# HydrogenSulfate/LFT

Hardware: AMD Instinct MI355X
Metric: LF patches/sec (5x5 angRes, 32x32 LR, 4xSR) (higher is better)
Workload: dtype bf16; 1 GPU; LFT 5x5 angRes 4xSR inference, batch=4 per GPU, 32x32 LR patches; global_batch=4, parallelism=dp1 (independent shards), streams_per_gpu=1, hip_graph=True, steps_in_flight=2

## Files before the change

### lft_amd/_lib.py

```python
from __future__ import annotations

import ctypes
import os
import subprocess
from ctypes import POINTER, c_char_p, c_float, c_int, c_longlong, c_size_t, c_void_p

HERE = os.path.dirname(os.path.abspath(__file__))
CSRC = os.path.join(HERE, "csrc")
LIB_PATH = os.environ.get("LFT_LIB_PATH") or os.path.join(HERE, "liblft_hip.so")
SOURCES = ["lft_api.hip", "lft_common.cuh", "lft_kernels_a.cuh", "lft_kernels_b.cuh", "lft_train.cuh", "lft_train_host.cuh", "lft_attn_maps.cuh", "lft_metrics.cuh", "lft_prepare.cuh"]
ABI_VERSION = 5
STATUS_NONFINITE = 1001

PREC_F32, PREC_BF16, PREC_F16 = 0, 1, 2
MATH_F32, MATH_BF16X3, MATH_BF16X6 = 0, 1, 2
NUM_PARAMS = 78

_lib = None


class LftError(RuntimeError):
    pass


# ... 75 lines not shown
    "lft_bicubic_fwd": (c_int, [c_void_p, c_void_p, c_int, c_int, c_int, c_int, c_int, c_void_p]),
    "lft_init_features_fwd": (c_int, [c_void_p, c_void_p, c_void_p, c_void_p, c_int, c_int, c_int, c_int, c_int, c_int, c_void_p]),
    "lft_ang_block_fwd": (c_int, [c_void_p, c_int, c_void_p, c_void_p, c_int, c_int, c_int, c_int, c_int, c_int, c_void_p]),
    "lft_spa_block_fwd": (c_int, [c_void_p, c_int, c_void_p, c_void_p, c_void_p, c_void_p, c_int, c_int, c_int, c_int, c_int, c_int, c_void_p]),
    "lft_upsample_fwd": (c_int, [c_void_p, c_void_p, c_void_p, c_void_p, c_void_p, c_int, c_int, c_int, c_int, c_int, c_int, c_void_p]),
    "lft_scene_counts": (c_int, [c_int, c_int, c_int, c_int, POINTER(c_int), POINTER(c_int)]),
    "lft_scene_divide": (c_int, [c_void_p, c_void_p, c_int, c_int, c_int, c_int, c_int, c_void_p]),
    "lft_scene_integrate": (c_int, [c_void_p, c_void_p, c_int, c_int, c_int, c_int, c_int, c_int, c_void_p]),
    "lft_train_tape_bytes": (c_int, [c_int, c_int, c_int, c_int, c_int, POINTER(c_size_t)]),
    "lft_train_grad_floats": (c_int, [c_int, POINTER(c_size_t)]),
    "lft_train_tape_offset": (c_int, [c_char_p, c_int, c_int, c_int, c_int, c_int, POINTER(c_size_t)]),
    "lft_train_forward": (c_int, [POINTER(c_void_p), c_int, c_void_p, c_void_p, c_void_p, c_int, c_int, c_int, c_int, c_int, c_int, c_void_p]),
    "lft_train_backward": (c_int, [POINTER(c_void_p), c_int, c_void_p, c_void_p, c_void_p, c_void_p, c_int, c_int, c_int, c_int, c_int, c_int, c_void_p]),
    "lft_train_backward_input": (c_int, [POINTER(c_void_p), c_int, c_void_p, c_void_p, c_void_p, c_void_p, c_void_p,
                                         c_int, c_int, c_int, c_int, c_int, c_int, c_void_p]),
    "lft_lr_grad_bwd": (c_int, [c_void_p, c_void_p, c_void_p, c_void_p, c_int, c_int, c_int, c_int, c_int, c_void_p]),
    "lft_train_backward_buckets": (c_int, [POINTER(c_void_p), c_int, c_void_p, c_void_p, c_void_p, c_void_p, c_int, c_int, c_int, c_int, c_int, c_int,
                                           c_void_p, c_void_p, c_void_p]),
    "lft_train_block_backward": (c_int, [POINTER(c_void_p), c_int, c_void_p, c_void_p, c_int, c_int, c_void_p, c_void_p, c_void_p,
                                         c_int, c_int, c_int, c_int, c_int, c_int, c_void_p]),
    "lft_train_grad_bucket": (c_int, [c_int, c_int, POINTER(c_size_t), POINTER(c_size_t)]),
    "lft_train_step_profiled": (c_int, [POINTER(c_void_p), c_int, c_void_p, c_void_p, c_void_p, c_void_p, c_void_p, c_int, c_int, c_int, c_int, c_int, c_int,
                                        c_void_p, c_int, POINTER(c_float), POINTER(c_char_p), POINTER(c_int)]),
    "lft_attn_maps_floats": (c_int, [c_int, c_int, c_int, c_int, c_int, c_int, POINTER(c_size_t)]),
    "lft_train_attn_maps": (c_int, [c_void_p, c_int, c_int, c_int, c_void_p, c_int, c_int, c_int, c_int, c_int, c_void_p]),
    "lft_l1_loss": (c_int, [c_void_p, c_void_p, c_longlong, c_void_p, c_float, c_void_p, c_void_p, c_void_p]),
    "lft_adam_step": (c_int, [c_void_p, c_void_p, c_void_p, c_void_p, c_longlong, c_float, c_float, c_float, c_float, c_int, c_float, c_float, c_void_p]),
    "lft_view_metrics_scratch_bytes": (c_int, [c_int, c_int, c_int, c_int, POINTER(c_size_t)]),
    "lft_view_metrics": (c_int, [c_void_p, c_void_p, c_int, c_int, c_int, c_int, c_float, c_void_p, c_void_p, c_void_p, c_void_p]),
    "lft_lf_prepare": (c_int, [c_void_p, c_int, c_int, c_int, c_int, c_int, c_int, POINTER(c_longlong), c_int, c_int,
                               POINTER(c_int), c_int, c_int, c_int, c_void_p, c_void_p, c_int, c_void_p, c_void_p, c_int,
                               c_void_p, c_void_p, c_void_p]),
    "lft_mfma_selftest": (c_int, [c_void_p, c_void_p, c_void_p, c_void_p, c_void_p, c_int, c_void_p]),
}
EXPORTS = tuple(_SIGS)
TEST_EXPORTS = ("lft_mfma_selftest",)
BLOCK_UPSAMPLE, BLOCK_SPA, BLOCK_ANG, BLOCK_INIT = 0, 1, 2, 3
LF_UINT8, LF_FLOAT32, LF_FLOAT64 = 0, 1, 2
MAPS_MEAN, MAPS_HEADS = 0, 1
GRAD_BUCKETS = 3
BUCKET_FN = ctypes.CFUNCTYPE(c_int, c_void_p, c_int, c_size_t, c_size_t)


def lib() -> ctypes.CDLL:
    global _lib
    if _lib is None:
        if not os.path.exists(LIB_PATH):
            raise LftError(f"{LIB_PATH} is missing: the HIP extension has not been built "
                           "(run __graft_entry__.build()); there is no CPU fallback")
        L = ctypes.CDLL(LIB_PATH)
        L.lft_version.restype, L.lft_version.argtypes = c_int, []
        got = L.lft_version()
        if got != ABI_VERSION:
            raise LftError(f"{LIB_PATH} reports ABI version {got}, this binding needs {ABI_VERSION}: rebuild it (__graft_entry__.build())")
        for name, (res, args) in _SIGS.items():
            fn = getattr(L, name)
            fn.restype, fn.argtypes = res, args
        _lib = L
    return _lib


def check(rc: int, what: str) -> None:
    if rc != 0:
        msg = lib().lft_last_error()
        raise LftError(f"{what} failed (code {rc}): {msg.decode() if msg else ''}")


def packed_bytes(A, h, w, s, prec) -> int:
    n = c_size_t(0)
    check(lib().lft_packed_bytes(A, h, w, s, prec, ctypes.byref(n)), "lft_packed_bytes")
    return n.value


def workspace_bytes(B, A, h, w, s, prec) -> int:
    n = c_size_t(0)
    check(lib().lft_workspace_bytes(B, A, h, w, s, prec, ctypes.byref(n)), "lft_workspace_bytes")
    return n.value
```

### lft_amd/csrc/lft_api.hip

```cpp
#include "../../include/lft_hip.h"
#include "../../include/lft_hip_test.h"
#include <hip/hip_runtime.h>
#include <stdint.h>

#include <cstdarg>
#include <cstdio>
#include <cmath>
#include <set>
#include <string>
#include <algorithm>
#include <type_traits>
#include <utility>
#include <vector>

#ifndef LFT_TU
#define LFT_TU 0
#endif

namespace {
#include "lft_kernels_a.cuh"
#include "lft_kernels_b.cuh"
#include "lft_metrics.cuh"
#include "lft_prepare.cuh"
#include "lft_train.cuh"
// ... 85 lines not shown
    return fail(LFT_ERR_ARG, "internal: no kernel variant for %d", (int)v);
}
template <int V> using int_c = std::integral_constant<int, V>;
template <typename F> int by_prec(int prec, F&& f) {
    if (prec == LFT_PREC_F32) return f(float{});
    if (prec == LFT_PREC_BF16) return f(bf16_t{});
    return f(f16_t{});
}
inline size_t align256(size_t x) { return (x + 255) & ~(size_t)255; }

struct Dims {
    int B, A, V, h, w, hw, s, gp, gt, nchunk;
    long long ntok;
};

int make_dims(int B, int A, int h, int w, int s, int prec, Dims* d) {
    if (prec != LFT_PREC_F32 && prec != LFT_PREC_BF16 && prec != LFT_PREC_F16)
        return fail(LFT_ERR_ARG, "prec must be LFT_PREC_F32, LFT_PREC_BF16 or LFT_PREC_F16, got %d", prec);
    if (B < 1 || A < 1 || h < 1 || w < 1) return fail(LFT_ERR_SHAPE, "B, A, h, w must be positive (B=%d A=%d h=%d w=%d)", B, A, h, w);
    if (s != 2 && s != 4) return fail(LFT_ERR_SHAPE, "scale factor must be 2 or 4, got %d", s);
    if (A * A > 128) return fail(LFT_ERR_UNSUPPORTED, "angRes %d (A*A=%d views > 128) is not implemented in this build", A, A * A);
    if ((long long)B * A * A * h * w > (1LL << 27)) return fail(LFT_ERR_SHAPE, "too many tokens");
    d->B = B; d->A = A; d->V = A * A; d->h = h; d->w = w; d->hw = h * w; d->s = s;
    d->gp = (s + 2) * (s + 2); d->gt = (d->gp + 31) / 32; d->nchunk = 2 * s * s;
    d->ntok = (long long)B * d->V * d->hw;
    return 0;
}

constexpr int kFragsConv = 72, kFragsAng = 64, kFragsSpa1 = 240, kFragsSpa1NoQ = 208, kFragsSpa2 = 176;
inline int frags_up(const Dims& d) { return d.nchunk * (4 + 2 * d.gt); }

struct PackedLayout {
    size_t conv0_w, ln_ang[kLayers], ln_spa[kLayers], ang_pe, petok[kLayers], spa_pe_img;
    size_t s_conv[3], s_ang[kLayers], s_spa1[kLayers], s_spa2[kLayers], s_up, total;
};

PackedLayout packed_layout(const Dims& d, int prec) {
    const size_t esz = prec == LFT_PREC_F32 ? 4 : 2, fragb = 64 * 8 * esz;
    PackedLayout L;
    size_t o = 0;
    auto take = [&](size_t bytes) { size_t r = o; o = align256(o + bytes); return r; };
    L.conv0_w = take(576 * 4);
    for (int l = 0; l < kLayers; ++l) { L.ln_ang[l] = take(256 * 4); L.ln_spa[l] = take(512 * 4); }
    L.ang_pe = take((size_t)((d.V + 31) / 32) * 2048 * 4);
    for (int l = 0; l < kLayers; ++l) L.petok[l] = take((size_t)((d.hw + 32 * kNwSpa1 - 1) / (32 * kNwSpa1)) * kNwSpa1 * 4096 * esz);
    L.spa_pe_img = take((size_t)d.hw * 64 * esz);
    for (int i = 0; i < 3; ++i) L.s_conv[i] = take(kFragsConv * fragb);
    for (int l = 0; l < kLayers; ++l) {
        L.s_ang[l] = take(kFragsAng * fragb);
        L.s_spa1[l] = take(kFragsSpa1 * fragb);
        L.s_spa2[l] = take(kFragsSpa2 * fragb);
    }
    L.s_up = take((size_t)frags_up(d) * fragb);
    L.total = o;
    return L;
}

struct WorkLayout {
    size_t x0, feat, xa, xb, tok, q, k, v, o, g, status, total;
};
WorkLayout work_layout(const Dims& d, int prec) {
    const size_t esz = prec == LFT_PREC_F32 ? 4 : 2;
    WorkLayout W;
    size_t o = 0;
    auto take = [&](size_t bytes) { size_t r = o; o = align256(o + bytes); return r; };
    const size_t n = (size_t)d.ntok;
    W.x0 = take(n * 64 * esz); W.feat = take(n * 64 * esz); W.xa = take(n * 64 * esz); W.xb = take(n * 64 * esz);
    W.tok = take(n * 128 * esz); W.q = take(n * 128 * esz); W.k = take(n * 128 * esz); W.v = take(n * 128 * esz);
    W.o = take(n * 128 * esz);
    W.g = take(n * d.gp * 4);
    W.status = take(256);
    W.total = o;
    return W;
}

template <typename T> size_t lds_conv64(int w) { return WRing<T, kConv64Chunk, kNwConv>::LDS_BYTES + ConvIn<T, kNwConv>::bytes(w) + kNwConv * TileIO<2, T>::BYTES + kConvZeroRow; }
constexpr size_t kLdsParams = 1024;
template <typename T, int CH = kSpaChunk> size_t lds_spa1(int w) {
    return WRing<T, CH, kNwSpa1>::LDS_BYTES + std::max<size_t>(ConvIn<T, kNwSpa1>::bytes(w), (size_t)kNwSpa1 * TileIO<4, T>::BYTES) + kLdsParams + kConvZeroRow;
}
template <typename T> size_t lds_spa2() { return WRing<T, kSpaChunk, kNwSpa2>::LDS_BYTES + kLdsParams + kNwSpa2 * TileIO<4, T>::BYTES; }
template <typename T> size_t lds_up() { return WRing<T, kUpChunk, kNwUp>::LDS_BYTES + kNwUp * TileIO<2, T>::BYTES; }
template <typename T> size_t lds_ang() { return (size_t)kFragsAng * 1024 * FragInfo<T>::PIECES + kLdsParams + 4 * TileIO<2, T>::BYTES; }
constexpr size_t kMaxLds = 160 * 1024;
template <typename K> int allow_lds(K kernel, size_t bytes, const char* name) {
    if (bytes > kMaxLds) return fail(LFT_ERR_SHAPE, "%s needs %zu B of LDS (> 160 KiB): view width too large for this build", name, bytes);
    if (bytes <= 64 * 1024) return 0;
    struct Done { int dev; const void* fn; size_t bytes; };
    static thread_local std::vector<Done> done;
    const void* fn = reinterpret_cast<const void*>(kernel);
    int dev = 0;
    LFT_HIP_OK(hipGetDevice(&dev));
    for (const auto& d : done)
        if (d.dev == dev && d.fn == fn && d.bytes >= bytes) return 0;
    LFT_HIP_OK(hipFuncSetAttribute(fn, hipFuncAttributeMaxDynamicSharedMemorySize, (int)bytes));
    done.push_back(Done{dev, fn, bytes});
    return 0;
}

template <typename P> P* at(const void* base, size_t off) { return reinterpret_cast<P*>(const_cast<char*>(static_cast<const char*>(base)) + off); }
inline unsigned blocks_for(long long items, int per_block) { return (unsigned)((items + per_block - 1) / per_block); }

PackOp lin_op(const float* src, int row0, int nrows, int ld, int k0, int ksteps, int kmap, float scale, int kmul = 1, int kadd = 0) {
    PackOp p{};
    p.src = src; p.kind = 0; p.row0 = row0; p.nrows = nrows; p.ntiles = (nrows + 31) / 32; p.ld = ld;
    p.kmul = kmul; p.kadd = kadd; p.k0 = k0; p.ksteps = ksteps; p.kmap = kmap; p.scale = scale; p.s = 0; p.frag0 = 0;
    return p;
}
void conv_ops(std::vector<PackOp>& v, const float* w, int nout) {
// ... 25 lines not shown
template <typename T> bool tok_lane_major(const Dims& d) {
    return d.hw % (32 * kNwSpa1) == 0 && (sizeof(T) == 4 || d.w % 32 == 0);
}
template <typename T, bool PE_ONLY>
int launch_spa1(unsigned nwg, const T* in, const T* ws, const float* ln, const T* petok, T* tok, T* q, T* k, T* v, T* pe_out,
                int nimg, const Dims& d, hipStream_t st, unsigned* status) {
    const size_t l16 = lds_spa1<T, 16>(d.w), l8 = lds_spa1<T, 8>(d.w);
    const size_t share = kMaxLds / kSpaOcc;
    const bool use8 = (l16 > share && l8 <= share) || l16 > kMaxLds;
    const bool lm = !PE_ONLY && tok_lane_major<T>(d);
    return dispatch<8, 16>(use8 ? 8 : 16, [&](auto CH) {
        return dispatch<true, false>(lm, [&](auto LM) {
            constexpr bool WQ = !(LM && sizeof(T) == 2);
            const size_t lds = CH == 8 ? l8 : l16;
            if (int rc = allow_lds(k_spa1<T, PE_ONLY, CH, LM, WQ>, lds, "k_spa1")) return rc;
            k_spa1<T, PE_ONLY, CH, LM, WQ><<<nwg, 64 * kNwSpa1, lds, st>>>(in, ws, ln, petok, tok, q, k, v, pe_out, nimg, d.h, d.w, status);
            return 0;
        });
    });
}

template <typename T>
int pack_impl(const float* const* P, void* packed, const Dims& d, int prec, hipStream_t st) {
    const PackedLayout L = packed_layout(d, prec);
    const float kAngScale = 0.35355339059327373f * LFT_LOG2E;
    const float kSpaScale = 0.25f * LFT_LOG2E;
    int rc;
    k_copy_f32<<<3, 256, 0, st>>>(P[0], at<float>(packed, L.conv0_w), 576);
    LFT_LAUNCH_OK("k_copy_f32");
    for (int i = 0; i < 3; ++i) {
        std::vector<PackOp> ops;
        conv_ops(ops, P[1 + i], 64);
        if ((rc = run_pack<T>(ops, at<T>(packed, L.s_conv[i]), kFragsConv, st))) return rc;
    }
    k_pe_tables<T><<<blocks_for(std::max<long long>((long long)((d.V + 31) / 32) * 2048, (long long)d.hw * 64), 256), 256, 0, st>>>(
        at<float>(packed, L.ang_pe), at<T>(packed, L.spa_pe_img), d.V, d.h, d.w);
    LFT_LAUNCH_OK("k_pe_tables");
    for (int l = 0; l < kLayers; ++l) {
        const float* const* q = P + 4 + 18 * l;
        float* lnS = at<float>(packed, L.ln_spa[l]);
        float* lnA = at<float>(packed, L.ln_ang[l]);
        const int srcS[4] = {1, 2, 5, 6}, srcA[4] = {10, 11, 14, 15};
        for (int j = 0; j < 4; ++j) {
            k_copy_f32<<<1, 256, 0, st>>>(q[srcS[j]], lnS + 128 * j, 128);
            k_copy_f32<<<1, 256, 0, st>>>(q[srcA[j]], lnA + 64 * j, 64);
        }
        LFT_LAUNCH_OK("k_copy_f32");
        {
            std::vector<PackOp> ops;
            ops.push_back(lin_op(q[12], 0, 64, 64, 0, 4, 1, kAngScale));
            ops.push_back(lin_op(q[12], 64, 64, 64, 0, 4, 1, 1.0f));
            ops.push_back(lin_op(q[12], 128, 64, 64, 0, 4, 1, 1.0f));
            ops.push_back(lin_op(q[13], 0, 64, 64, 0, 4, 1, 1.0f));
            ops.push_back(lin_op(q[16], 0, 128, 64, 0, 4, 1, 1.0f));
            ops.push_back(lin_op(q[17], 0, 64, 128, 0, 8, 1, 1.0f));
            if ((rc = run_pack<T>(ops, at<T>(packed, L.s_ang[l]), kFragsAng, st))) return rc;
        }
        {
            std::vector<PackOp> ops;
            conv_ops(ops, q[0], 128);
            ops.push_back(lin_op(q[3], 256, 128, 128, 0, 8, 1, 1.0f));
            ops.push_back(lin_op(q[3], 128, 128, 128, 0, 8, 1, 1.0f));
            ops.push_back(lin_op(q[3], 0, 128, 128, 0, 8, 1, kSpaScale));
            if ((rc = run_pack<T>(ops, at<T>(packed, L.s_spa1[l]), kFragsSpa1, st))) return rc;
        }
        {
// ... 1 lines not shown
            ops.push_back(lin_op(q[4], 0, 128, 128, 0, 8, (sizeof(T) == 2 && tok_lane_major<T>(d)) ? 1 : 0, 1.0f));
            for (int c = 0; c < 4; ++c) {
                ops.push_back(lin_op(q[7], 64 * c, 64, 128, 0, 8, 1, 1.0f));
                ops.push_back(lin_op(q[8], 0, 128, 256, 64 * c, 4, 1, 1.0f));
            }
            ops.push_back(lin_op(q[9], 0, 64, 128, 0, 8, 1, 1.0f));
            if ((rc = run_pack<T>(ops, at<T>(packed, L.s_spa2[l]), kFragsSpa2, st))) return rc;
        }
        if ((rc = launch_spa1<T, true>((unsigned)((d.hw + 32 * kNwSpa1 - 1) / (32 * kNwSpa1)), at<T>(packed, L.spa_pe_img), at<T>(packed, L.s_spa1[l]), nullptr, nullptr,
                                       nullptr, nullptr, nullptr, nullptr, at<T>(packed, L.petok[l]), 1, d, st, nullptr))) return rc;
        LFT_LAUNCH_OK("k_spa1<pe>");
    }
    {
        std::vector<PackOp> ops;
        for (int c = 0; c < d.nchunk; ++c) {
            ops.push_back(lin_op(P[76], 32 * c, 32, 64, 0, 4, 1, 1.0f));
            PackOp m = lin_op(P[77], 0, d.gp, 0, 32 * c, 2, 1, 1.0f);
            m.kind = 1; m.s = d.s; m.ntiles = d.gt;
            ops.push_back(m);
        }
        if ((rc = run_pack<T>(ops, at<T>(packed, L.s_up), frags_up(d), st))) return rc;
    }
    return 0;
}

void launch_assemble(const float* lr, const float* g, float* out, int B, int A, int h, int w, int s, hipStream_t st, int gld = 0, unsigned* status = nullptr) {
    const dim3 tg((unsigned)((A * w + 7) / 8) * (unsigned)((A * h + 7) / 8) * (unsigned)B);
    if (!gld) gld = (s + 2) * (s + 2);
    if (s == 2) k_assemble_t<2><<<tg, 256, 0, st>>>(lr, g, out, B, A, h, w, gld, status);
    else k_assemble_t<4><<<tg, 256, 0, st>>>(lr, g, out, B, A, h, w, gld, status);
}

template <typename T>
int init_features(const void* packed, const PackedLayout& L, const float* lr, T* x0, T* ta, T* tb, T* feat, const Dims& d, hipStream_t st) {
    const int nimg = d.B * d.V, nwg = nimg * ((d.hw + 32 * kNwConv - 1) / (32 * kNwConv));
    const size_t lds = lds_conv64<T>(d.w);
    int rc;
    if ((rc = allow_lds(k_conv64<T, false>, lds, "k_conv64"))) return rc;
    if ((rc = allow_lds(k_conv64<T, true>, lds, "k_conv64"))) return rc;
    k_conv0<T><<<dim3((unsigned)((d.hw + kConv0Tok - 1) / kConv0Tok), (unsigned)nimg), 256, 0, st>>>(lr, at<float>(packed, L.conv0_w), x0, d.B, d.A, d.h, d.w);
    LFT_LAUNCH_OK("k_conv0");
    k_conv64<T, false><<<nwg, 64 * kNwConv, lds, st>>>(x0, ta, nullptr, at<T>(packed, L.s_conv[0]), nimg, d.h, d.w);
    LFT_LAUNCH_OK("k_conv64");
    k_conv64<T, false><<<nwg, 64 * kNwConv, lds, st>>>(ta, tb, nullptr, at<T>(packed, L.s_conv[1]), nimg, d.h, d.w);
    LFT_LAUNCH_OK("k_conv64");
    k_conv64<T, true><<<nwg, 64 * kNwConv, lds, st>>>(tb, feat, x0, at<T>(packed, L.s_conv[2]), nimg, d.h, d.w);
    LFT_LAUNCH_OK("k_conv64");
    return 0;
}
template <typename T, int CT, int LL>
int ang_multi(const void* packed, const PackedLayout& L, int l, const T* in, T* out, const Dims& d, hipStream_t st, unsigned* status) {
    constexpr bool WLDS = sizeof(T) == 2;
    constexpr int NG = (sizeof(T) == 2 && CT <= 3) ? 2 : 1;
    constexpr size_t FB = 1024 * FragInfo<T>::PIECES;
    const size_t lds = (WLDS ? 64 * FB : 0) + 1024 + (size_t)NG * CT * 8 * FB + (size_t)NG * CT * TileIO<2, T>::BYTES;
    const int npix = d.B * d.hw;
    int rc;
    const unsigned grid = std::min<unsigned>(blocks_for(npix, NG), 256u * (unsigned)std::max<size_t>(1, kMaxLds / lds));
    if ((rc = allow_lds(k_ang_multi<T, CT, WLDS, NG, LL>, lds, "k_ang_multi"))) return rc;
    k_ang_multi<T, CT, WLDS, NG, LL><<<grid, 64 * CT * NG, lds, st>>>(in, out, at<T>(packed, L.s_ang[l]), at<float>(packed, L.ln_ang[l]),
                                                                     at<float>(packed, L.ang_pe), d.V, d.hw, npix, status);
    LFT_LAUNCH_OK("k_ang");
    return 0;
}
template <typename T>
int ang_block(const void* packed, const PackedLayout& L, int l, const T* in, T* out, const Dims& d, hipStream_t st, unsigned* status = nullptr) {
    auto multi = [&](auto CT, auto LL) { return ang_multi<T, CT, LL>(packed, L, l, in, out, d, st, status); };
    if (d.V > 100) return multi(int_c<4>{}, int_c<13>{});
    if (d.V > 96) return multi(int_c<4>{}, int_c<9>{});
    if (d.V > 64) return multi(int_c<3>{}, int_c<9>{});
    if (d.V == 64) return multi(int_c<2>{}, int_c<16>{});
    if (d.V > 32) return multi(int_c<2>{}, int_c<9>{});
    const int npix = d.B * d.hw;
    const size_t lds = lds_ang<T>();
    int rc;
    const unsigned grid = std::min<unsigned>(blocks_for(npix, 4), 256u * (unsigned)std::max<size_t>(1, kMaxLds / lds));
    if ((rc = allow_lds(k_ang<T, 13>, lds, "k_ang"))) return rc;
    k_ang<T, 13><<<grid, 256, lds, st>>>(in, out, at<T>(packed, L.s_ang[l]), at<float>(packed, L.ln_ang[l]),
                                         at<float>(packed, L.ang_pe), d.V, d.hw, npix, status);
    LFT_LAUNCH_OK("k_ang");
    return 0;
// ... 79 lines not shown
}

template <typename T>
int forward_impl(const void* packed, const float* lr, float* out, void* ws, const Dims& d, int prec, hipStream_t st) {
    const PackedLayout L = packed_layout(d, prec);
    const WorkLayout W = work_layout(d, prec);
    T *x0 = at<T>(ws, W.x0), *feat = at<T>(ws, W.feat), *xa = at<T>(ws, W.xa), *xb = at<T>(ws, W.xb);
    int rc;
    if ((rc = init_features<T>(packed, L, lr, x0, xa, xb, feat, d, st))) return rc;
    const T* cur = feat;
    for (int l = 0; l < kLayers; ++l) {
        if ((rc = ang_block<T>(packed, L, l, cur, xa, d, st, at<unsigned>(ws, W.status)))) return rc;
        const bool last = l == kLayers - 1;
        if ((rc = spa_block<T>(packed, L, l, xa, last ? feat : nullptr, xb, ws, W, d, st, last && tok_lane_major<T>(d)))) return rc;
        cur = xb;
    }
    return upsample<T>(packed, L, xb, lr, out, ws, W, d, st, tok_lane_major<T>(d));
}

template <typename T>
int kernel_time_impl(const char* name, const void* packed, void* ws, const Dims& d, int prec, int reps, hipStream_t st, float* ms_out) {
    const PackedLayout L = packed_layout(d, prec);
    const WorkLayout W = work_layout(d, prec);
    T *x0 = at<T>(ws, W.x0), *feat = at<T>(ws, W.feat), *xa = at<T>(ws, W.xa), *xb = at<T>(ws, W.xb);
    const std::string k(name);
    auto once = [&]() -> int {
        if (k == "k_ang") return ang_block<T>(packed, L, 1, xb, xa, d, st, at<unsigned>(ws, W.status));
        if (k == "k_spa1") return spa_part_a<T>(packed, L, 1, xa, ws, W, d, st);
        if (k == "k_spa_b" || k == "k_spa_attn+k_spa2") return spa_part_b<T>(packed, L, 1, nullptr, xb, ws, W, d, st);
        if (k == "k_conv64") {
            const int nimg = d.B * d.V, nwg = nimg * ((d.hw + 32 * kNwConv - 1) / (32 * kNwConv));
            const size_t lds = lds_conv64<T>(d.w);
            int rc;
            if ((rc = allow_lds(k_conv64<T, false>, lds, "k_conv64"))) return rc;
            k_conv64<T, false><<<nwg, 64 * kNwConv, lds, st>>>(x0, feat, nullptr, at<T>(packed, L.s_conv[0]), nimg, d.h, d.w);
            LFT_LAUNCH_OK("k_conv64");
            return 0;
        }
        return fail(LFT_ERR_ARG, "lft_kernel_time: unknown kernel %s", name);
    };
    int rc;
    if ((rc = once())) return rc;
    hipEvent_t e0, e1;
    LFT_HIP_OK(hipEventCreate(&e0));
    LFT_HIP_OK(hipEventCreate(&e1));
    LFT_HIP_OK(hipEventRecord(e0, st));
    for (int i = 0; i < reps && !rc; ++i) rc = once();
    LFT_HIP_OK(hipEventRecord(e1, st));
    LFT_HIP_OK(hipEventSynchronize(e1));
    float ms = 0.0f;
    LFT_HIP_OK(hipEventElapsedTime(&ms, e0, e1));
    (void)hipEventDestroy(e0); (void)hipEventDestroy(e1);
    if (rc) return rc;
    *ms_out = ms / (float)reps;
    return 0;
}
#include "lft_train_host.cuh"

}

extern "C" {

#if LFT_TU != 2
int lft_version(void) { return LFT_ABI_VERSION; }
const char* lft_last_error(void) { return g_err; }

int lft_packed_bytes(int A, int h, int w, int s, int prec, size_t* out_bytes) {
    Dims d; int rc;
// ... 58 lines not shown
                        [&] { return lft_forward(packed, lr, out, workspace, B, A, h, w, s, prec, stream); });
}

int lft_kernel_time(const char* kernel, const void* packed, void* workspace, int B, int A, int h, int w, int s, int prec, int reps,
                    void* stream, float* ms_out) {
    Dims d; int rc;
    if (!kernel || !packed || !workspace || !ms_out || reps < 1) return fail(LFT_ERR_ARG, "bad argument");
    if ((rc = make_dims(B, A, h, w, s, prec, &d))) return rc;
    hipStream_t st = static_cast<hipStream_t>(stream);
    return by_prec(prec, [&](auto t) { using T = decltype(t); return kernel_time_impl<T>(kernel, packed, workspace, d, prec, reps, st, ms_out); });
}

int lft_bicubic_fwd(const float* lr, float* out, int B, int A, int h, int w, int s, void* stream) {
    Dims d; int rc;
    if (!lr || !out) return fail(LFT_ERR_ARG, "null pointer");
    if ((rc = make_dims(B, A, h, w, s, LFT_PREC_F32, &d))) return rc;
    const dim3 grid((unsigned)((A * w * s + 255) / 256), (unsigned)(A * h * s), (unsigned)B);
    k_bicubic<<<grid, 256, 0, static_cast<hipStream_t>(stream)>>>(lr, out, B, A, h, w, s);
    LFT_LAUNCH_OK("k_bicubic");
    return 0;
}

int lft_init_features_fwd(const void* packed, const float* lr, void* act_out, void* workspace, int B, int A, int h, int w, int s,
                          int prec, void* stream) {
    Dims d; int rc;
    if (!packed || !lr || !act_out || !workspace) return fail(LFT_ERR_ARG, "null pointer");
    if ((rc = make_dims(B, A, h, w, s, prec, &d))) return rc;
    const PackedLayout L = packed_layout(d, prec);
    const WorkLayout W = work_layout(d, prec);
    hipStream_t st = static_cast<hipStream_t>(stream);
    return by_prec(prec, [&](auto t) {
        using T = decltype(t);
        return init_features<T>(packed, L, lr, at<T>(workspace, W.x0), at<T>(workspace, W.xa), at<T>(workspace, W.xb), static_cast<T*>(act_out), d, st);
    });
}

int lft_ang_block_fwd(const void* packed, int layer, const void* act_in, void* act_out, int B, int A, int h, int w, int s, int prec,
                      void* stream) {
    Dims d; int rc;
    if (!packed || !act_in || !act_out) return fail(LFT_ERR_ARG, "null pointer");
    if (layer < 0 || layer >= kLayers) return fail(LFT_ERR_ARG, "layer %d out of range", layer);
    if ((rc = make_dims(B, A, h, w, s, prec, &d))) return rc;
    const PackedLayout L = packed_layout(d, prec);
    hipStream_t st = static_cast<hipStream_t>(stream);
    return by_prec(prec, [&](auto t) {
        using T = decltype(t);
        return ang_block<T>(packed, L, layer, static_cast<const T*>(act_in), static_cast<T*>(act_out), d, st);
    });
}

int lft_spa_block_fwd(const void* packed, int layer, const void* act_in, const void* skip, void* act_out, void* workspace, int B, int A,
                      int h, int w, int s, int prec, void* stream) {
    Dims d; int rc;
    if (!packed || !act_in || !act_out || !workspace) return fail(LFT_ERR_ARG, "null pointer");
    if (layer < 0 || layer >= kLayers) return fail(LFT_ERR_ARG, "layer %d out of range", layer);
    if ((rc = make_dims(B, A, h, w, s, prec, &d))) return rc;
    const PackedLayout L = packed_layout(d, prec);
    const WorkLayout W = work_layout(d, prec);
    hipStream_t st = static_cast<hipStream_t>(stream);
    return by_prec(prec, [&](auto t) {
        using T = decltype(t);
        return spa_block<T>(packed, L, layer, static_cast<const T*>(act_in), static_cast<const T*>(skip), static_cast<T*>(act_out), workspace, W, d, st);
    });
}

int lft_upsample_fwd(const void* packed, const void* act_in, const float* lr, float* out, void* workspace, int B, int A, int h, int w,
// ... 325 lines not shown
```

### lft_amd/csrc/lft_kernels_a.cuh

```cuda
#pragma once
#include "lft_common.cuh"

struct PackOp {
    const float* src;
    int kind, row0, nrows, ntiles, ld, kmul, kadd, k0, ksteps, kmap, frag0, s;
    float scale;
    int order;
};
__host__ __device__ __forceinline__ int wfrag_index(int OT, int KS, int ot, int ks) {
    const int g = ot >> 2, G = OT - 4 * g < 4 ? OT - 4 * g : 4;
    return 4 * g * KS + ks * G + (ot & 3);
}
__host__ __device__ __forceinline__ void wfrag_coords(int OT, int KS, int lf, int order, int& nt, int& ks) {
    if (!order) { nt = lf / KS; ks = lf % KS; return; }
    const int gl = (OT - 1) >> 2, g = lf / (4 * KS) < gl ? lf / (4 * KS) : gl, G = OT - 4 * g < 4 ? OT - 4 * g : 4, rem = lf - 4 * g * KS;
    ks = rem / G; nt = 4 * g + rem % G;
}
constexpr int LFT_PACK_MAXOPS = 40;
struct PackArgs {
    int nops;
    PackOp op[LFT_PACK_MAXOPS];
};

LFT_DEV float upm_entry(const float* __restrict__ w3, int n, int kk, int s) {
// ... 155 lines not shown
LFT_DEV void clear_zero_row(char* zero_row) {
    if (threadIdx.x < kConvZeroRow / 16) store_raw16(zero_row + threadIdx.x * 16, raw16{0u, 0u, 0u, 0u});
}
template <int NT, typename T, int NW, typename Ring>
LFT_DEV void conv3x3_tile(const char* lds_in, const char* zero_row, int tl, int y, int x, bool ok, int h, int w, int hh,
                          Ring& ring, f32x16 (&acc)[NT]) {
    using CI = ConvIn<T, NW>;
    static_assert(CI::ROW_BYTES <= kConvZeroRow, "zero row too short");
#pragma unroll
    for (int tap = 0; tap < 9; ++tap) {
        const int dy = tap / 3 - 1, dx = tap % 3 - 1;
        const int yy = y + dy, xx = x + dx;
        const bool inb = ok && yy >= 0 && yy < h && xx >= 0 && xx < w;
        const int slot = tl + w + 1 + dy * w + dx;
        const char* row = inb ? lds_in + slot * CI::ROW_BYTES : zero_row;
        const int sw = inb ? CI::swz(slot) : 0;
#pragma unroll
        for (int ks = 0; ks < 4; ++ks) {
            Frag<T> b;
            if constexpr (sizeof(T) == 2) {
                b.v = __builtin_bit_cast(typename H16<T>::v8, load_raw16(row + (((2 * ks + hh) ^ sw) * 16)));
            } else {
                b.lo = __builtin_bit_cast(f32x4, load_raw16(row + (((4 * ks + 2 * hh) ^ sw) * 16)));
                b.hi = __builtin_bit_cast(f32x4, load_raw16(row + (((4 * ks + 2 * hh + 1) ^ sw) * 16)));
            }
#pragma unroll
            for (int nt = 0; nt < NT; ++nt) mma(ring.next(), b, acc[nt]);
        }
    }
}

constexpr int kNwConv = 4;
constexpr int kConv64Chunk = 12;
template <typename T, bool RES, int NW = kNwConv>
__global__ __launch_bounds__(64 * NW) void k_conv64(const T* __restrict__ in, T* __restrict__ out, const T* __restrict__ res,
                                                   const T* __restrict__ wstream, int nimg, int h, int w) {
    extern __shared__ __attribute__((aligned(16))) char smem[];
    constexpr int TT = 32 * NW;
    const int lane = threadIdx.x & 63, r = lane & 31, hh = lane >> 5, wave = threadIdx.x >> 6;
    const int hw = h * w, tpi = (hw + TT - 1) / TT;
    const int bid = xcd_tile(blockIdx.x, gridDim.x);
    const int im = bid / tpi, p0 = (bid % tpi) * TT;
    const int tl = wave * 32 + r, p = p0 + tl;
    const bool ok = p < hw;
    const int t0 = p0 + wave * 32, nvalid = max(0, min(32, hw - t0));
    const size_t tile_off = ((size_t)im * hw + min(t0, hw - 1)) * 64;
    char* lds_in = smem + WRing<T, kConv64Chunk, NW>::LDS_BYTES;
    char* scr = lds_in + ConvIn<T, NW>::bytes(w) + wave * TileIO<2, T>::BYTES;
    char* zero_row = lds_in + ConvIn<T, NW>::bytes(w) + NW * TileIO<2, T>::BYTES;
    f32x16 rr[2];
    if (RES) load_tile<2, T>(res + tile_off, nvalid, lane, rr, scr);
    WRing<T, kConv64Chunk, NW> ring;
    ring.init(wstream, smem, 72);
    stage_conv_input<T, NW>(in + (size_t)im * hw * 64, p0, hw, w, lds_in);
    clear_zero_row(zero_row);
    wait_staged();
    __syncthreads();
    LFT_NOTE_ASM_("USE", kNoteConvIn, 0);
    f32x16 acc[2];
    zero_acc<2>(acc);
    conv3x3_tile<2, T, NW>(lds_in, zero_row, tl, p / w, p % w, ok, h, w, hh, ring, acc);
#pragma unroll
    for (int nt = 0; nt < 2; ++nt)
#pragma unroll
        for (int i = 0; i < 16; ++i) acc[nt][i] = lrelu02_fast(acc[nt][i]);
    if (RES) {
#pragma unroll
        for (int nt = 0; nt < 2; ++nt) acc[nt] += rr[nt];
    }
    store_tile<2, T>(out + tile_off, nvalid, lane, acc, scr);
}

template <int NT_OUT, int KS, typename T>
LFT_DEV void linear_lds(const char* wl, int f0, int lane, const Frag<T> (&x)[KS], f32x16 (&y)[NT_OUT]) {
#pragma unroll
    for (int nt = 0; nt < NT_OUT; ++nt)
#pragma unroll
        for (int ks = 0; ks < KS; ++ks)
            mma(frag_from_pieces(wl + (f0 + nt * KS + ks) * 1024 * FragInfo<T>::PIECES, lane, T()), x[ks], y[nt]);
}

template <typename T, int NLIVE = 16>
__global__ __launch_bounds__(256, 2) void k_ang(const T* __restrict__ X, T* __restrict__ Y, const T* __restrict__ ws,
                                             const float* __restrict__ ln, const float* __restrict__ pe,
                                             int V, int hw, int npix, unsigned* __restrict__ status) {
    extern __shared__ __attribute__((aligned(16))) char smem[];
    constexpr int FB = 1024 * FragInfo<T>::PIECES;
    const int lane = threadIdx.x & 63, r = lane & 31, hh = lane >> 5;
    const int wave = __builtin_amdgcn_readfirstlane(threadIdx.x >> 6);
    unsigned bad = 0;
    {
        const char* g = reinterpret_cast<const char*>(ws);
        LFT_NOTE_ASM_("DMA", kNoteAngW, 0);
#pragma unroll
        for (int i = 0; i < 16 * FragInfo<T>::PIECES; ++i) {
            const int piece = wave * 16 * FragInfo<T>::PIECES + i;
            glds_piece(g + piece * 1024, smem + piece * 1024, lane);
        }
    }
    float* lds_ln = reinterpret_cast<float*>(smem + 64 * FB);
    LFT_STAMP(0);
    const raw16 lnv = params_load(ln, 256);
    asm volatile("s_waitcnt vmcnt(0)" ::: "memory");
// ... 256 lines not shown
```

Baseline: 9869 patches/s.

## Fuse conv_init0 into conv_init1 via composed weights and recompute residual

For 16-bit precisions, the first 1->64 conv and the second 64->64 conv are algebraically composed into a 96-wide (81 used) weight matrix, so a new kernel builds conv1's output directly from staged LR pixels with MFMA. The third conv recomputes the conv0 residual from LR in-kernel instead of reading a stored x0. Two launches and the x0/ta round trips through global memory go away. The cost is extra LDS and the composed-weight MFMA, and numerics differ because conv0's intermediate rounding is skipped and the composed weights use an f16 operand type.

```diff
diff --git a/lft_amd/_lib.py b/lft_amd/_lib.py
--- a/lft_amd/_lib.py
+++ b/lft_amd/_lib.py
@@ -131,9 +131,11 @@
                                POINTER(c_int), c_int, c_int, c_int, c_void_p, c_void_p, c_int, c_void_p, c_void_p, c_int,
                                c_void_p, c_void_p, c_void_p]),
     "lft_mfma_selftest": (c_int, [c_void_p, c_void_p, c_void_p, c_void_p, c_void_p, c_int, c_void_p]),
+    "lft_init_features_legacy_fwd": (c_int, [c_void_p, c_void_p, c_void_p, c_void_p, c_int, c_int, c_int, c_int, c_int, c_int, c_void_p]),
+    "lft_conv0_fwd": (c_int, [c_void_p, c_void_p, c_void_p, c_int, c_int, c_int, c_int, c_int, c_int, c_int, c_void_p]),
 }
 EXPORTS = tuple(_SIGS)
-TEST_EXPORTS = ("lft_mfma_selftest",)
+TEST_EXPORTS = ("lft_mfma_selftest", "lft_init_features_legacy_fwd", "lft_conv0_fwd")
 BLOCK_UPSAMPLE, BLOCK_SPA, BLOCK_ANG, BLOCK_INIT = 0, 1, 2, 3
 LF_UINT8, LF_FLOAT32, LF_FLOAT64 = 0, 1, 2
 MAPS_MEAN, MAPS_HEADS = 0, 1
@@ -153,6 +155,8 @@
         if got != ABI_VERSION:
             raise LftError(f"{LIB_PATH} reports ABI version {got}, this binding needs {ABI_VERSION}: rebuild it (__graft_entry__.build())")
         for name, (res, args) in _SIGS.items():
+            if name in TEST_EXPORTS and not hasattr(L, name):
+                continue
             fn = getattr(L, name)
             fn.restype, fn.argtypes = res, args
         _lib = L
diff --git a/lft_amd/csrc/lft_api.hip b/lft_amd/csrc/lft_api.hip
--- a/lft_amd/csrc/lft_api.hip
+++ b/lft_amd/csrc/lft_api.hip
@@ -141,6 +141,7 @@
 
 struct PackedLayout {
     size_t conv0_w, ln_ang[kLayers], ln_spa[kLayers], ang_pe, petok[kLayers], spa_pe_img;
+    size_t w01, s_w01;
     size_t s_conv[3], s_ang[kLayers], s_spa1[kLayers], s_spa2[kLayers], s_up, total;
 };
 
@@ -154,7 +155,11 @@
     L.ang_pe = take((size_t)((d.V + 31) / 32) * 2048 * 4);
     for (int l = 0; l < kLayers; ++l) L.petok[l] = take((size_t)((d.hw + 32 * kNwSpa1 - 1) / (32 * kNwSpa1)) * kNwSpa1 * 4096 * esz);
     L.spa_pe_img = take((size_t)d.hw * 64 * esz);
-    for (int i = 0; i < 3; ++i) L.s_conv[i] = take(kFragsConv * fragb);
+    const bool lp = prec != LFT_PREC_F32;
+    L.w01 = take(lp ? 64 * kW01K * 4 : 0);
+    L.s_conv[0] = take(kFragsConv * fragb);
+    L.s_w01 = take(lp ? kW01Frags * fragb : 0);
+    for (int i = 1; i < 3; ++i) L.s_conv[i] = take(kFragsConv * fragb);
     for (int l = 0; l < kLayers; ++l) {
         L.s_ang[l] = take(kFragsAng * fragb);
         L.s_spa1[l] = take(kFragsSpa1 * fragb);
@@ -184,6 +189,7 @@
 }
 
 template <typename T> size_t lds_conv64(int w) { return WRing<T, kConv64Chunk, kNwConv>::LDS_BYTES + ConvIn<T, kNwConv>::bytes(w) + kNwConv * TileIO<2, T>::BYTES + kConvZeroRow; }
+template <typename T> size_t lds_conv64_lr(int w) { return lds_conv64<T>(w) + std::max<size_t>(LrStage<kNwConv>::bytes(w), kConv0WBytes); }
 constexpr size_t kLdsParams = 1024;
 template <typename T, int CH = kSpaChunk> size_t lds_spa1(int w) {
     return WRing<T, CH, kNwSpa1>::LDS_BYTES + std::max<size_t>(ConvIn<T, kNwSpa1>::bytes(w), (size_t)kNwSpa1 * TileIO<4, T>::BYTES) + kLdsParams + kConvZeroRow;
@@ -275,6 +281,12 @@
         std::vector<PackOp> ops;
         conv_ops(ops, P[1 + i], 64);
         if ((rc = run_pack<T>(ops, at<T>(packed, L.s_conv[i]), kFragsConv, st))) return rc;
+    }
+    if constexpr (sizeof(T) == 2) {
+        k_compose_w01<<<blocks_for(64 * kW01K, 256), 256, 0, st>>>(P[0], P[1], at<float>(packed, L.w01));
+        LFT_LAUNCH_OK("k_compose_w01");
+        std::vector<PackOp> ops{lin_op(at<float>(packed, L.w01), 0, 64, kW01K, 0, kW01K / 16, 0, 1.0f)};
+        if ((rc = run_pack<ConvLrOp>(ops, at<ConvLrOp>(packed, L.s_w01), kW01Frags, st))) return rc;
     }
     k_pe_tables<T><<<blocks_for(std::max<long long>((long long)((d.V + 31) / 32) * 2048, (long long)d.hw * 64), 256), 256, 0, st>>>(
         at<float>(packed, L.ang_pe), at<T>(packed, L.spa_pe_img), d.V, d.h, d.w);
@@ -342,21 +354,39 @@
 }
 
 template <typename T>
-int init_features(const void* packed, const PackedLayout& L, const float* lr, T* x0, T* ta, T* tb, T* feat, const Dims& d, hipStream_t st) {
+int init_features_x0(const void* packed, const PackedLayout& L, const float* lr, T* x0, T* ta, T* tb, T* feat, const Dims& d, hipStream_t st) {
     const int nimg = d.B * d.V, nwg = nimg * ((d.hw + 32 * kNwConv - 1) / (32 * kNwConv));
     const size_t lds = lds_conv64<T>(d.w);
     int rc;
-    if ((rc = allow_lds(k_conv64<T, false>, lds, "k_conv64"))) return rc;
-    if ((rc = allow_lds(k_conv64<T, true>, lds, "k_conv64"))) return rc;
+    if ((rc = allow_lds(k_conv64<T, 0>, lds, "k_conv64"))) return rc;
+    if ((rc = allow_lds(k_conv64<T, 1>, lds, "k_conv64"))) return rc;
     k_conv0<T><<<dim3((unsigned)((d.hw + kConv0Tok - 1) / kConv0Tok), (unsigned)nimg), 256, 0, st>>>(lr, at<float>(packed, L.conv0_w), x0, d.B, d.A, d.h, d.w);
     LFT_LAUNCH_OK("k_conv0");
-    k_conv64<T, false><<<nwg, 64 * kNwConv, lds, st>>>(x0, ta, nullptr, at<T>(packed, L.s_conv[0]), nimg, d.h, d.w);
+    k_conv64<T, 0><<<nwg, 64 * kNwConv, lds, st>>>(x0, ta, nullptr, at<T>(packed, L.s_conv[0]), nimg, d.h, d.w, ConvLr{});
     LFT_LAUNCH_OK("k_conv64");
-    k_conv64<T, false><<<nwg, 64 * kNwConv, lds, st>>>(ta, tb, nullptr, at<T>(packed, L.s_conv[1]), nimg, d.h, d.w);
+    k_conv64<T, 0><<<nwg, 64 * kNwConv, lds, st>>>(ta, tb, nullptr, at<T>(packed, L.s_conv[1]), nimg, d.h, d.w, ConvLr{});
     LFT_LAUNCH_OK("k_conv64");
-    k_conv64<T, true><<<nwg, 64 * kNwConv, lds, st>>>(tb, feat, x0, at<T>(packed, L.s_conv[2]), nimg, d.h, d.w);
+    k_conv64<T, 1><<<nwg, 64 * kNwConv, lds, st>>>(tb, feat, x0, at<T>(packed, L.s_conv[2]), nimg, d.h, d.w, ConvLr{});
     LFT_LAUNCH_OK("k_conv64");
     return 0;
+}
+template <typename T>
+int init_features(const void* packed, const PackedLayout& L, const float* lr, T* x0, T* ta, T* tb, T* feat, const Dims& d, hipStream_t st) {
+    if constexpr (sizeof(T) == 4) return init_features_x0<T>(packed, L, lr, x0, ta, tb, feat, d, st);
+    else {
+        const int nimg = d.B * d.V, nwg = nimg * ((d.hw + 32 * kNwConv - 1) / (32 * kNwConv));
+        const size_t lds = lds_conv64_lr<T>(d.w);
+        int rc;
+        if (L.s_w01 + kW01Frags * 1024 != L.s_conv[1]) return fail(LFT_ERR_ARG, "internal: W01 fragments are not in front of conv_init.2's stream");
+        if ((rc = allow_lds(k_conv64_lr<T>, lds, "k_conv64"))) return rc;
+        if ((rc = allow_lds(k_conv64<T, 2>, lds, "k_conv64"))) return rc;
+        k_conv64_lr<T><<<nwg, 64 * kNwConv, lds, st>>>(lr, tb, at<T>(packed, L.s_w01), d.A, nimg, d.h, d.w);
+        LFT_LAUNCH_OK("k_conv64");
+        k_conv64<T, 2><<<nwg, 64 * kNwConv, lds, st>>>(tb, feat, nullptr, at<T>(packed, L.s_conv[2]), nimg, d.h, d.w,
+                                                      ConvLr{lr, at<float>(packed, L.conv0_w), d.A});
+        LFT_LAUNCH_OK("k_conv64");
+        return 0;
+    }
 }
 template <typename T, int CT, int LL>
 int ang_multi(const void* packed, const PackedLayout& L, int l, const T* in, T* out, const Dims& d, hipStream_t st, unsigned* status) {
@@ -502,8 +532,8 @@
             const int nimg = d.B * d.V, nwg = nimg * ((d.hw + 32 * kNwConv - 1) / (32 * kNwConv));
             const size_t lds = lds_conv64<T>(d.w);
             int rc;
-            if ((rc = allow_lds(k_conv64<T, false>, lds, "k_conv64"))) return rc;
-            k_conv64<T, false><<<nwg, 64 * kNwConv, lds, st>>>(x0, feat, nullptr, at<T>(packed, L.s_conv[0]), nimg, d.h, d.w);
+            if ((rc = allow_lds(k_conv64<T, 0>, lds, "k_conv64"))) return rc;
+            k_conv64<T, 0><<<nwg, 64 * kNwConv, lds, st>>>(xb, x0, nullptr, at<T>(packed, L.s_conv[0]), nimg, d.h, d.w, ConvLr{});
             LFT_LAUNCH_OK("k_conv64");
             return 0;
         }
@@ -628,6 +658,44 @@
     return by_prec(prec, [&](auto t) {
         using T = decltype(t);
         return init_features<T>(packed, L, lr, at<T>(workspace, W.x0), at<T>(workspace, W.xa), at<T>(workspace, W.xb), static_cast<T*>(act_out), d, st);
+    });
+}
+
+int lft_init_features_legacy_fwd(const void* packed, const float* lr, void* act_out, void* workspace, int B, int A, int h, int w, int s,
+                                 int prec, void* stream) {
+    Dims d; int rc;
+    if (!packed || !lr || !act_out || !workspace) return fail(LFT_ERR_ARG, "null pointer");
+    if ((rc = make_dims(B, A, h, w, s, prec, &d))) return rc;
+    const PackedLayout L = packed_layout(d, prec);
+    const WorkLayout W = work_layout(d, prec);
+    hipStream_t st = static_cast<hipStream_t>(stream);
+    return by_prec(prec, [&](auto t) {
+        using T = decltype(t);
+        return init_features_x0<T>(packed, L, lr, at<T>(workspace, W.x0), at<T>(workspace, W.xa), at<T>(workspace, W.xb), static_cast<T*>(act_out), d, st);
+    });
+}
+
+int lft_conv0_fwd(const void* packed, const float* lr, void* x0_out, int recomputed, int B, int A, int h, int w, int s, int prec, void* stream) {
+    Dims d; int rc;
+    if (!packed || !lr || !x0_out) return fail(LFT_ERR_ARG, "null pointer");
+    if ((rc = make_dims(B, A, h, w, s, prec, &d))) return rc;
+    if (recomputed && prec == LFT_PREC_F32) return fail(LFT_ERR_ARG, "conv_init0 is recomputed in the 16-bit precisions only");
+    const PackedLayout L = packed_layout(d, prec);
+    hipStream_t st = static_cast<hipStream_t>(stream);
+    return by_prec(prec, [&](auto t) {
+        using T = decltype(t);
+        const int nimg = d.B * d.V;
+        const float* w0 = at<float>(packed, L.conv0_w);
+        if constexpr (sizeof(T) == 2) {
+            if (recomputed) {
+                k_conv0_recomputed<T><<<nimg * ((d.hw + 32 * kNwConv - 1) / (32 * kNwConv)), 64 * kNwConv, 0, st>>>(static_cast<T*>(x0_out), nimg, d.h, d.w, ConvLr{lr, w0, d.A});
+                LFT_LAUNCH_OK("k_conv0_recomputed");
+                return 0;
+            }
+        }
+        k_conv0<T><<<dim3((unsigned)((d.hw + kConv0Tok - 1) / kConv0Tok), (unsigned)nimg), 256, 0, st>>>(lr, w0, static_cast<T*>(x0_out), d.B, d.A, d.h, d.w);
+        LFT_LAUNCH_OK("k_conv0");
+        return 0;
     });
 }
 
diff --git a/lft_amd/csrc/lft_kernels_a.cuh b/lft_amd/csrc/lft_kernels_a.cuh
--- a/lft_amd/csrc/lft_kernels_a.cuh
+++ b/lft_amd/csrc/lft_kernels_a.cuh
@@ -211,9 +211,77 @@
 
 constexpr int kNwConv = 4;
 constexpr int kConv64Chunk = 12;
-template <typename T, bool RES, int NW = kNwConv>
+
+typedef f16_t ConvLrOp;
+constexpr int kW01K = 96, kW01Frags = 12;
+__host__ __device__ __forceinline__ int conv01_row_channel(int rho) { return (rho & ~12) | ((rho & 4) << 1) | ((rho & 8) >> 1); }
+__global__ void k_compose_w01(const float* __restrict__ w0, const float* __restrict__ w1, float* __restrict__ w01) {
+    const int idx = blockIdx.x * blockDim.x + threadIdx.x;
+    if (idx >= 64 * kW01K) return;
+    const int rho = idx / kW01K, k = idx - rho * kW01K;
+    float v = 0.0f;
+    if (k < 81) {
+        const int o = conv01_row_channel(rho), t1 = k / 9, t0 = k - 9 * t1;
+        for (int c = 0; c < 64; ++c) v += w1[o * 576 + c * 9 + t1] * w0[c * 9 + t0];
+    }
+    w01[idx] = v;
+}
+LFT_DEV const float* lr_view(const float* __restrict__ lr, int im, int A, int h, int w) {
+    const int V = A * A, b = im / V, v = im - b * V, a1 = v / A, a2 = v - a1 * A;
+    return lr + (size_t)b * (A * h) * (A * w) + (size_t)(a1 * h) * (A * w) + a2 * w;
+}
+template <int NW> struct LrStage {
+    static __host__ __device__ int width(int w) { return w + 4; }
+    static __host__ __device__ int max_rows(int w) { return (32 * NW + 2 * w + 1) / w + 6; }
+    static __host__ __device__ int bytes(int w) { return (max_rows(w) * width(w) * 4 + 15) & ~15; }
+};
+constexpr int kConv0WBytes = 9 * 64 * 4;
+LFT_DEV void conv0_w_stage(const float* __restrict__ w0, float* wl) {
+    float wv[3];
+#pragma unroll
+    for (int k = 0; k < 3; ++k) wv[k] = w0[min((int)threadIdx.x + 256 * k, 575)];
+#pragma unroll
+    for (int k = 0; k < 3; ++k) {
+        const int i = (int)threadIdx.x + 256 * k, ch = i / 9, t = i - ch * 9;
+        if (i < 576) wl[t * 64 + ch] = wv[k];
+    }
+}
+LFT_DEV void conv0_taps_load(const float* __restrict__ img, int ldi, int y, int x, int h, int w, float (&val)[9]) {
+#pragma unroll
+    for (int t = 0; t < 9; ++t) {
+        const int yy = y + t / 3 - 1, xx = x + t % 3 - 1;
+        val[t] = img[min(max(yy, 0), h - 1) * ldi + min(max(xx, 0), w - 1)];
+    }
+}
+template <typename T>
+LFT_DEV void conv0_token_acc(const float (&tap)[9], const float* wl, int y, int x, int h, int w, int hh, f32x16 (&rr)[2]) {
+    float val[9];
+#pragma unroll
+    for (int t = 0; t < 9; ++t) {
+        const int yy = y + t / 3 - 1, xx = x + t % 3 - 1;
+        val[t] = (yy >= 0 && yy < h && xx >= 0 && xx < w) ? tap[t] : 0.0f;
+    }
+#pragma unroll
+    for (int nt = 0; nt < 2; ++nt)
+#pragma unroll
+        for (int g = 0; g < 4; ++g) {
+            f32x4 wq[9];
+#pragma unroll
+            for (int t = 0; t < 9; ++t) wq[t] = __builtin_bit_cast(f32x4, load_raw16(reinterpret_cast<const char*>(wl + t * 64 + 32 * nt + 8 * g + 4 * hh)));
+#pragma unroll
+            for (int j = 0; j < 4; ++j) {
+                float a = 0.0f;
+#pragma unroll
+                for (int t = 0; t < 9; ++t) a += wq[t][j] * val[t];
+                rr[nt][4 * g + j] = (float)(T)a;
+            }
+        }
+}
+struct ConvLr { const float* lr; const float* w0; int A; };
+
+template <typename T, int RES, int NW = kNwConv>
 __global__ __launch_bounds__(64 * NW) void k_conv64(const T* __restrict__ in, T* __restrict__ out, const T* __restrict__ res,
-                                                   const T* __restrict__ wstream, int nimg, int h, int w) {
+                                                   const T* __restrict__ wstream, int nimg, int h, int w, ConvLr cl) {
     extern __shared__ __attribute__((aligned(16))) char smem[];
     constexpr int TT = 32 * NW;
     const int lane = threadIdx.x & 63, r = lane & 31, hh = lane >> 5, wave = threadIdx.x >> 6;
@@ -227,15 +295,21 @@
     char* lds_in = smem + WRing<T, kConv64Chunk, NW>::LDS_BYTES;
     char* scr = lds_in + ConvIn<T, NW>::bytes(w) + wave * TileIO<2, T>::BYTES;
     char* zero_row = lds_in + ConvIn<T, NW>::bytes(w) + NW * TileIO<2, T>::BYTES;
+    float* wl = reinterpret_cast<float*>(zero_row + kConvZeroRow);
+    const int pc = min(p, hw - 1), yc = pc / w, xc = pc - yc * w;
     f32x16 rr[2];
-    if (RES) load_tile<2, T>(res + tile_off, nvalid, lane, rr, scr);
+    float tap[9];
+    if constexpr (RES == 1) load_tile<2, T>(res + tile_off, nvalid, lane, rr, scr);
+    if constexpr (RES == 2) conv0_taps_load(lr_view(cl.lr, im, cl.A, h, w), cl.A * w, yc, xc, h, w, tap);
     WRing<T, kConv64Chunk, NW> ring;
     ring.init(wstream, smem, 72);
     stage_conv_input<T, NW>(in + (size_t)im * hw * 64, p0, hw, w, lds_in);
     clear_zero_row(zero_row);
+    if constexpr (RES == 2) conv0_w_stage(cl.w0, wl);
     wait_staged();
     __syncthreads();
     LFT_NOTE_ASM_("USE", kNoteConvIn, 0);
+    if constexpr (RES == 2) conv0_token_acc<T>(tap, wl, yc, xc, h, w, hh, rr);
     f32x16 acc[2];
     zero_acc<2>(acc);
     conv3x3_tile<2, T, NW>(lds_in, zero_row, tl, p / w, p % w, ok, h, w, hh, ring, acc);
@@ -243,11 +317,120 @@
     for (int nt = 0; nt < 2; ++nt)
 #pragma unroll
         for (int i = 0; i < 16; ++i) acc[nt][i] = lrelu02_fast(acc[nt][i]);
-    if (RES) {
+    if constexpr (RES != 0) {
 #pragma unroll
         for (int nt = 0; nt < 2; ++nt) acc[nt] += rr[nt];
     }
     store_tile<2, T>(out + tile_off, nvalid, lane, acc, scr);
+}
+
+template <typename T, int NW = kNwConv>
+__global__ __launch_bounds__(64 * NW) void k_conv64_lr(const float* __restrict__ lr, T* __restrict__ out, const T* __restrict__ wstream,
+                                                      int A, int nimg, int h, int w) {
+    static_assert(sizeof(T) == 2, "16-bit operand types only");
+    extern __shared__ __attribute__((aligned(16))) char smem[];
+    using CI = ConvIn<T, NW>;
+    constexpr int TT = 32 * NW;
+    const int lane = threadIdx.x & 63, r = lane & 31, hh = lane >> 5, wave = __builtin_amdgcn_readfirstlane(threadIdx.x >> 6);
+    const int hw = h * w, tpi = (hw + TT - 1) / TT;
+    const int bid = xcd_tile(blockIdx.x, gridDim.x);
+    const int im = bid / tpi, p0 = (bid % tpi) * TT;
+    const int tl = wave * 32 + r, p = p0 + tl;
+    const bool ok = p < hw;
+    const int t0 = p0 + wave * 32, nvalid = max(0, min(32, hw - t0));
+    const size_t tile_off = ((size_t)im * hw + min(t0, hw - 1)) * 64;
+    char* lds_in = smem + WRing<T, kConv64Chunk, NW>::LDS_BYTES;
+    char* scr = lds_in + CI::bytes(w) + wave * TileIO<2, T>::BYTES;
+    char* zero_row = lds_in + CI::bytes(w) + NW * TileIO<2, T>::BYTES;
+    float* lrs = reinterpret_cast<float*>(zero_row + kConvZeroRow);
+    WRing<T, kConv64Chunk, NW> ring;
+    ring.init(wstream, smem, kW01Frags + 72);
+    const int nslots = CI::slots(w), LW = LrStage<NW>::width(w);
+    const int y_first = max(p0 - w - 1, 0) / w, y_last = min(p0 + TT + w, hw - 1) / w;
+    {
+        const float* img = lr_view(lr, im, A, h, w);
+        const int n = (y_last - y_first + 5) * LW, ldi = A * w;
+        for (int i = threadIdx.x; i < n; i += 64 * NW) {
+            const int row = i / LW, yy = y_first - 2 + row, xx = i - row * LW - 2;
+            const float v = img[min(max(yy, 0), h - 1) * ldi + min(max(xx, 0), w - 1)];
+            lrs[i] = (yy >= 0 && yy < h && xx >= 0 && xx < w) ? v : 0.0f;
+        }
+    }
+    clear_zero_row(zero_row);
+    Frag<ConvLrOp> wf[kW01Frags];
+#pragma unroll
+    for (int i = 0; i < kW01Frags; ++i) wf[i].v = __builtin_bit_cast(H16<ConvLrOp>::v8, ring.next().v);
+    for (int ct = wave; ct * 32 < nslots; ct += NW) {
+        const int slot = ct * 32 + r;
+        const int q = min(max(p0 - w - 1 + slot, 0), hw - 1), y = q / w, x = q - y * w;
+        const float* pl = lrs + (y - y_first) * LW + x;
+        float P[5][5];
+#pragma unroll
+        for (int a = 0; a < 5; ++a)
+#pragma unroll
+            for (int b = 0; b < 5; ++b) P[a][b] = pl[a * LW + b];
+        bool m[9];
+#pragma unroll
+        for (int t = 0; t < 9; ++t) {
+            const int yy = y + t / 3 - 1, xx = x + t % 3 - 1;
+            m[t] = yy >= 0 && yy < h && xx >= 0 && xx < w;
+        }
+        auto masked = [&](int k) -> float {
+            if (k >= 81) return 0.0f;
+            const int t1 = k / 9, t0 = k % 9;
+            return m[t1] ? P[t1 / 3 + t0 / 3][t1 % 3 + t0 % 3] : 0.0f;
+        };
+        f32x16 a01[2];
+        zero_acc<2>(a01);
+#pragma unroll
+        for (int ks = 0; ks < kW01K / 16; ++ks) {
+            Frag<ConvLrOp> b;
+#pragma unroll
+            for (int j = 0; j < 8; ++j) b.v[j] = (ConvLrOp)(hh ? masked(16 * ks + 8 + j) : masked(16 * ks + j));
+#pragma unroll
+            for (int nt = 0; nt < 2; ++nt) mma(wf[nt * (kW01K / 16) + ks], b, a01[nt]);
+        }
+#pragma unroll
+        for (int nt = 0; nt < 2; ++nt)
+#pragma unroll
+            for (int i = 0; i < 16; ++i) a01[nt][i] = lrelu02_fast(a01[nt][i]);
+        Frag<T> of[4];
+        acc_frags<2, T>(a01, of);
+        if (slot < nslots) {
+            char* row = lds_in + slot * CI::ROW_BYTES;
+            const int sw = CI::swz(slot);
+#pragma unroll
+            for (int ks = 0; ks < 4; ++ks) store_raw16(row + (((2 * ks + hh) ^ sw) * 16), __builtin_bit_cast(raw16, of[ks].v));
+        }
+    }
+    wg_barrier_keep_vm();
+    f32x16 acc[2];
+    zero_acc<2>(acc);
+    conv3x3_tile<2, T, NW>(lds_in, zero_row, tl, p / w, p % w, ok, h, w, hh, ring, acc);
+#pragma unroll
+    for (int nt = 0; nt < 2; ++nt)
+#pragma unroll
+        for (int i = 0; i < 16; ++i) acc[nt][i] = lrelu02_fast(acc[nt][i]);
+    store_tile<2, T>(out + tile_off, nvalid, lane, acc, scr);
+}
+template <typename T, int NW = kNwConv>
+__global__ __launch_bounds__(64 * NW) void k_conv0_recomputed(T* __restrict__ out, int nimg, int h, int w, ConvLr cl) {
+    __shared__ __attribute__((aligned(16))) char sm[kConv0WBytes + NW * TileIO<2, T>::BYTES];
+    constexpr int TT = 32 * NW;
+    const int lane = threadIdx.x & 63, r = lane & 31, hh = lane >> 5, wave = threadIdx.x >> 6;
+    const int hw = h * w, tpi = (hw + TT - 1) / TT;
+    const int im = blockIdx.x / tpi, p0 = (blockIdx.x % tpi) * TT;
+    const int t0 = p0 + wave * 32, nvalid = max(0, min(32, hw - t0));
+    const size_t tile_off = ((size_t)im * hw + min(t0, hw - 1)) * 64;
+    const int pc = min(p0 + wave * 32 + r, hw - 1), yc = pc / w, xc = pc - yc * w;
+    float* wl = reinterpret_cast<float*>(sm);
+    float tap[9];
+    conv0_taps_load(lr_view(cl.lr, im, cl.A, h, w), cl.A * w, yc, xc, h, w, tap);
+    conv0_w_stage(cl.w0, wl);
+    __syncthreads();
+    f32x16 rr[2];
+    conv0_token_acc<T>(tap, wl, yc, xc, h, w, hh, rr);
+    store_tile<2, T>(out + tile_off, nvalid, lane, rr, sm + kConv0WBytes + wave * TileIO<2, T>::BYTES);
 }
 
 template <int NT_OUT, int KS, typename T>
```

Measured after the change: 10200 patches/s (median of 6 runs). 3.4% higher.
